# Jiraiya812/Fast-CU-Decision-HEVC

Measured on AMD Instinct MI355X. Metric: CTUs/sec (RDO decision only) at 4K all-intra, higher is better.
Workload: dtype int32+f64

## Files before the change

### __graft_entry__.py

```python
import importlib.util
import os
import subprocess
import sys

ROOT = os.path.dirname(os.path.abspath(__file__))
PKG_DIR = os.path.join(ROOT, "fast-cu-decision-hevc_amd")
PKG_NAME = "fast_cu_decision_hevc_amd"


def load_package():
    if PKG_NAME in sys.modules:
        return sys.modules[PKG_NAME]
    spec = importlib.util.spec_from_file_location(PKG_NAME, os.path.join(PKG_DIR, "__init__.py"),
                                                  submodule_search_locations=[PKG_DIR])
    mod = importlib.util.module_from_spec(spec)
    sys.modules[PKG_NAME] = mod
    spec.loader.exec_module(mod)
    return mod


REQUIRED_FLAG = "-amdgpu-remove-redundant-endcf=false"
ENGINE_FLAGS = ["--offload-arch=gfx950", "-std=c++17", "-O3", "-ffp-contract=off", "-fPIC", "-shared",
                "-DFCU_WAVES_PER_EU=4", "-Wno-unused-value", "-mllvm", REQUIRED_FLAG]

# ... 31 lines not shown
    hipcc = os.environ.get("HIPCC", "/opt/rocm/bin/hipcc")
    digest = _stale(lib, [p for p in srcs if not p.endswith("__graft_entry__.py")], ENGINE_FLAGS)
    if digest is not None:
        _run([hipcc] + ENGINE_FLAGS + ['-DFCU_BUILD_FLAGS="%s"' % " ".join(ENGINE_FLAGS),
                        "-o", lib, os.path.join(csrc, "fcu_kernels.hip")], csrc)
        with open(lib + ".stamp", "w") as f:
            f.write(digest)
        import ctypes
        info = ctypes.CDLL(lib).fcu_build_info
        info.restype = ctypes.c_char_p
        if REQUIRED_FLAG not in info().decode():
            raise RuntimeError("libfcu.so was built without %s: %s" % (REQUIRED_FLAG, info().decode()))
    _run(["make", "-s"], os.path.join(ROOT, "oracle"))
    emu = os.path.join(ROOT, "tests", "emu")
    shared = [p for p in [os.path.join(emu, "picture_emu.h")] if os.path.exists(p)]
    for name in ("fcu_emu", "dbk_emu", "sao_emu", "wpp_emu", "tiles_emu", "lf_tiles_emu", "lf_slices_emu", "report_emu", "host_emu", "hash_emu", "maps_emu", "labels_emu", "cu_trace_emu"):
        if not os.path.exists(os.path.join(emu, name + ".cpp")):
            continue
        if _newer(os.path.join(emu, "lib%s.so" % name), srcs + shared + [os.path.join(emu, name + ".cpp")]):
            _run(["g++", "-std=c++17", "-O2", "-fPIC", "-ffp-contract=off", "-shared", "-o", "lib%s.so" % name, name + ".cpp"], emu)
    orc = os.path.join(ROOT, "oracle")
    ref_srcs = [os.path.join(emu, "lf_tile_ref.c")] + [os.path.join(orc, f) for f in ("hmo_sao.c", "hmo_tables.c", "hmo.h", "hmo_int.h")]
    if _newer(os.path.join(emu, "liblf_tile_ref.so"), ref_srcs):
        _run(["gcc", "-O2", "-std=c11", "-fPIC", "-ffp-contract=off", "-fno-fast-math", "-shared", "-o", "liblf_tile_ref.so",
              "lf_tile_ref.c", os.path.join(orc, "hmo_tables.c"), "-lm"], emu)
    ref_srcs = [os.path.join(emu, "lf_slice_ref.c")] + [os.path.join(orc, f) for f in ("hmo_sao.c", "hmo_deblock.c", "hmo_tables.c", "hmo.h", "hmo_int.h")]
    if os.path.exists(ref_srcs[0]) and _newer(os.path.join(emu, "liblf_slice_ref.so"), ref_srcs):
        _run(["gcc", "-O2", "-std=c11", "-fPIC", "-ffp-contract=off", "-fno-fast-math", "-shared", "-o", "liblf_slice_ref.so",
              "lf_slice_ref.c", os.path.join(orc, "hmo_tables.c"), "-lm"], emu)
    ref_mk = os.path.join(ROOT, "oracle", "ref", "build_ref.sh")
    if os.path.isdir("/root/reference") and os.path.exists(ref_mk):
# ... 60 lines not shown
```

### fast-cu-decision-hevc_amd/csrc/fcu_engine.h

```cpp
#pragma once
#include <stdint.h>
#include <string.h>
#include <type_traits>
#include "../../include/fcu.h"

#ifdef FCU_EMU
#include <math.h>
#include <stdio.h>
#include <stdlib.h>
#define FCU_DEV static inline
#define FCU_MEMBER inline
#define FCU_NOINLINE
#define FCU_INLINE
#define FCU_TABLE static const
static int g_emu_phase = 0, g_emu_in_phase = 0, g_emu_lane = 0, g_emu_relax = 0;
#define FCU_EMU_RELAX(on) (g_emu_relax = (on))
static inline int fcu_emu_phase_begin() { g_emu_phase++; g_emu_in_phase = 1; g_emu_lane = 0; return 0; }
static inline int fcu_emu_phase_next(int lane) { if (lane + 1 >= 64) g_emu_in_phase = 0; g_emu_lane = lane + 1; return lane + 1; }
template <class T> static inline T fcu_emu_uni(T v, int site, int line)
{
  enum { SITES = 2048, K = 32, B = 16 };
  struct Seen { int phase, first, cur, idx, n; unsigned char vals[K][B]; };
  static Seen seen[SITES];
  if (g_emu_in_phase && !g_emu_relax && sizeof(T) <= B && site < SITES) {
    Seen &s = seen[site];
    if (s.phase != g_emu_phase) { s.phase = g_emu_phase; s.first = s.cur = g_emu_lane; s.idx = 0; s.n = 0; }
    if (s.cur != g_emu_lane) { s.cur = g_emu_lane; s.idx = 0; }
    if (g_emu_lane == s.first) { if (s.n < K) memcpy(s.vals[s.n++], &v, sizeof(T)); }
    else if (s.idx < s.n && memcmp(s.vals[s.idx], &v, sizeof(T)) != 0) { fprintf(stderr, "FCU_UNI at line %d: value differs between lanes of one phase\n", line); abort(); }
    s.idx++;
  }
  return v;
}
#define FCU_FOR_LANES for (int lane = fcu_emu_phase_begin(); lane < 64; lane = fcu_emu_phase_next(lane))
#define FCU_ATOMIC_ADD(p, v) (*(p) += (v))
#define FCU_ATOMIC_MAX(p, v) do { if (*(p) < (v)) *(p) = (v); } while (0)
#define FCU_ATOMIC_OR(p, v) (*(p) |= (v))
#define FCU_WAVE_ADD(p, v) (*(p) += (v))
#define FCU_WAVE_MIN64(p, v) do { if ((v) < *(p)) *(p) = (v); } while (0)
#define FCU_IN_LDS(p) do { } while (0)
#define FCU_UNI(x) fcu_emu_uni((x), __COUNTER__, __LINE__)
#define FCU_HBM
#define FCU_FLOOR(x) floor(x)
#define FCU_CHECK(c) do { if (!(c)) { fprintf(stderr, "FCU_CHECK failed: %s (line %d)\n", #c, __LINE__); abort(); } } while (0)
static unsigned long long g_emu_cu_paths[3] = { 0, 0, 0 };
#else
#define FCU_DEV __device__ static
#define FCU_MEMBER __device__ inline
#define FCU_NOINLINE __noinline__
#define FCU_INLINE __attribute__((always_inline))
#define FCU_TABLE __device__ static const
#define FCU_FOR_LANES for (int lane = (int)threadIdx.x, fcu_once_ = 1; fcu_once_; fcu_once_ = 0, __syncthreads())
#define FCU_ATOMIC_ADD(p, v) atomicAdd((p), (v))
#define FCU_ATOMIC_MAX(p, v) atomicMax((p), (v))
#define FCU_ATOMIC_OR(p, v) atomicOr((p), (v))
__device__ inline uint32_t fcu_wave_sum(uint32_t v)
{
  v += (uint32_t)__builtin_amdgcn_update_dpp(0, (int)v, 0xb1, 0xf, 0xf, false);
  v += (uint32_t)__builtin_amdgcn_update_dpp(0, (int)v, 0x4e, 0xf, 0xf, false);
  v += (uint32_t)__builtin_amdgcn_update_dpp(0, (int)v, 0x124, 0xf, 0xf, false);
  v += (uint32_t)__builtin_amdgcn_update_dpp(0, (int)v, 0x128, 0xf, 0xf, false);
  v += (uint32_t)__builtin_amdgcn_update_dpp(0, (int)v, 0x142, 0xa, 0xf, false);
  v += (uint32_t)__builtin_amdgcn_update_dpp(0, (int)v, 0x143, 0xc, 0xf, false);
  return (uint32_t)__builtin_amdgcn_readlane((int)v, 63);
}
__device__ inline unsigned long long fcu_wave_min64(unsigned long long v)
{
// ... 43 lines not shown
#define FCU_TOC(E_, v, idx) do { if ((idx) == 10 && threadIdx.x == 0) (E_).C->prof[idx] += (unsigned long long)(clock64() - v); } while (0)
#define FCU_COUNT(E_, idx, n) do { } while (0)
#elif defined(FCU_PROFILE_RDOQ) || defined(FCU_PROFILE_DEPTH)
#define FCU_TOC(E_, v, idx) do { if ((idx) < 11 && threadIdx.x == 0) (E_).C->prof[idx] += (unsigned long long)(clock64() - v); } while (0)
#define FCU_COUNT(E_, idx, n) do { } while (0)
#elif defined(FCU_PROFILE_RMD)
#define FCU_MTOC(E_, v, idx) do { if (threadIdx.x == 0) (E_).C->prof[idx] += (unsigned long long)(clock64() - v); } while (0)
#define FCU_TOC(E_, v, idx) do { if ((idx) < 11 && threadIdx.x == 0) (E_).C->prof[idx] += (unsigned long long)(clock64() - v); } while (0)
#define FCU_COUNT(E_, idx, n) do { } while (0)
#elif defined(FCU_PROFILE_CUSYN)
#define FCU_STOC(E_, v, idx) do { if (threadIdx.x == 0) (E_).C->prof[idx] += (unsigned long long)(clock64() - v); } while (0)
#define FCU_SPATH(E_, path) do { if (threadIdx.x == 0) (E_).C->prof[15] += 1ull << (21 * (path)); } while (0)
#define FCU_S7_COEFF(E_, v, comp) do { if (g_S.prof_s7 == 1) FCU_STOC(E_, v, (comp) ? 14 : 13); } while (0)
#define FCU_TOC(E_, v, idx) do { if ((idx) < 11 && threadIdx.x == 0) (E_).C->prof[idx] += (unsigned long long)(clock64() - v); } while (0)
#define FCU_COUNT(E_, idx, n) do { } while (0)
#else
#define FCU_TOC(E_, v, idx) do { if (threadIdx.x == 0) (E_).C->prof[idx] += (unsigned long long)(clock64() - v); } while (0)
#define FCU_COUNT(E_, idx, n) do { (E_).C->prof[idx] += (unsigned long long)(n); } while (0)
#endif
#else
#define FCU_TIC(v) do { } while (0)
#define FCU_TOC(E_, v, idx) do { } while (0)
#define FCU_COUNT(E_, idx, n) do { } while (0)
#endif
#ifndef FCU_QTOC
#define FCU_QTIC(v) do { } while (0)
#define FCU_QTOC(E_, v, idx) do { } while (0)
#endif
#ifndef FCU_ITOC
#define FCU_ITOC(E_, v, idx) do { } while (0)
#endif
#ifndef FCU_MTOC
#define FCU_MTOC(E_, v, idx) do { } while (0)
#endif
#ifndef FCU_STOC
#define FCU_STOC(E_, v, idx) do { } while (0)
#define FCU_SPATH(E_, path) do { } while (0)
#define FCU_S7_COEFF(E_, v, comp) do { } while (0)
#endif

#include "fcu_tables.h"

struct HotTables { uint32_t bin[256]; uint16_t scan[3][16]; uint8_t scan_cg8[3][4]; uint8_t ctx_ind_map4x4[16]; uint8_t group_idx[32];
                   uint64_t scan4_nib[3], map4_nib; uint32_t cnt_bits[4]; };
#ifdef FCU_EMU
static HotTables g_hot;
#else
__shared__ HotTables g_hot;
// ... 322 lines not shown
  }
  return first + offset;
}
FCU_DEV int coef_remain_bins(uint32_t symbol, uint32_t rparam)
{
  int code = (int)symbol;
  if (code < (3 << rparam)) return (int)(((uint32_t)code >> rparam) + 1) + (int)rparam;
  uint32_t length = rparam;
  code -= 3 << rparam;
  while (code >= (1 << length)) code -= 1 << (length++);
  return (int)(3 + length + 1 - rparam) + (int)length;
}
#ifdef FCU_EMU
enum { WALK_RDOQ_CALLS, WALK_RDOQ_TOP_IS_GROUP0, WALK_RDOQ_AHEAD_GROUPS, WALK_RDOQ_ONLY_GROUP0, WALK_RDOQ_ONLY_LAST_GROUP, WALK_RDOQ_ALL_ZERO,
       WALK_BITS_CALLS, WALK_BITS_ONE_EMPTY_RUN_BETWEEN, WALK_BITS_SECOND_ROUND, WALK_N };
extern "C" { __attribute__((weak)) unsigned long long fcu_emu_walk_cnt[WALK_N]; }
static const int32_t *g_emu_lscan_lo = nullptr, *g_emu_lscan_hi = nullptr;
#define FCU_WALK_COUNT(i, n) (fcu_emu_walk_cnt[i] += (unsigned long long)(n))
#define FCU_CHECK_LSCAN(p) FCU_CHECK((const int32_t *)(p) >= g_emu_lscan_lo && (const int32_t *)(p) < g_emu_lscan_hi)
#else
#define FCU_WALK_COUNT(i, n) do { } while (0)
#define FCU_CHECK_LSCAN(p) do { } while (0)
#endif
template <int SER>
FCU_DEV FCU_INLINE void code_coeff_body(int c, const int16_t *coef, int st, int last, int log2, int comp, int scanType, int tsFlag, const Params &P_, int16_t *absCoeff)
{
  if (SER) { c = FCU_UNI(c); coef = FCU_UNI(coef); last = FCU_UNI(last); scanType = FCU_UNI(scanType); tsFlag = FCU_UNI(tsFlag); absCoeff = FCU_UNI(absCoeff); }
  const Params &P = *FCU_UNI(&P_);
  st = FCU_UNI(st); log2 = FCU_UNI(log2); comp = FCU_UNI(comp);
  FCU_IN_LDS(absCoeff);
  const FCU_HBM int16_t *coefg = (const FCU_HBM int16_t *)coef;
  const int ch = comp ? 1 : 0, N = 1 << log2; int n2 = N * N;
  if (last < 0 && st == 1 && n2 >= 64) {
    int q = (n2 >> 6) - 1;
    for (; q >= 0; q--) {
      uint32_t w[32];
// ... 556 lines not shown
    for (int sp = 0; sp < n2 - 16; sp++) other |= dstg[sp * st];
    FCU_WALK_COUNT(WALK_RDOQ_ONLY_LAST_GROUP, !other);
  }
#endif
  return rdoq_finish<SER>(cb, P, srcg, dstg, recg, cgg, st, log2, ch, scanType, cbfCtx, scan, scanCG, cgflag, cgLastScanPos, lastScanPos, baseCost, blockUncodedCost, lambda);
}

#ifdef FCU_EMU
template <class T> struct LaneVar {
  T v[64];
  LaneVar() { for (int i = 0; i < 64; i++) v[i] = T(); }
  void set(int lane, T x) { v[lane] = x; }
  T own(int lane) const { return v[lane]; }
  T get(int k) const { return v[k]; }
  void put(int k, T x) { v[k] = x; }
};
FCU_DEV uint32_t lane_mask16(const LaneVar<int> &f) { uint32_t m = 0; for (int k = 0; k < 16; k++) m |= (uint32_t)(f.v[k] != 0) << k; return m; }
#else
#if defined(__HIP_DEVICE_COMPILE__)
#define FCU_READLANE(v, k) __builtin_amdgcn_readlane((v), (k))
#define FCU_WRITELANE(val_, k_, old_) (((int)threadIdx.x == (k_)) ? (val_) : (old_))
#define FCU_BALLOT(p) __builtin_amdgcn_ballot_w64(p)
#else
#define FCU_READLANE(v, k) (v)
#define FCU_WRITELANE(val_, k_, old_) (val_)
#define FCU_BALLOT(p) ((unsigned long long)(p))
#endif
template <class T> struct LaneVar;
template <> struct LaneVar<int> {
  int r = 0;
  __device__ void set(int, int x) { r = x; }
  __device__ int own(int) const { return r; }
  __device__ int get(int k) const { return FCU_READLANE(r, k); }
  __device__ void put(int k, int x) { r = FCU_WRITELANE(x, k, r); }
};
template <> struct LaneVar<double> {
  double r = 0;
  __device__ void set(int, double x) { r = x; }
  __device__ double own(int) const { return r; }
  __device__ double get(int k) const
  { union { double d; int i[2]; } u; u.d = r; u.i[0] = FCU_READLANE(u.i[0], k); u.i[1] = FCU_READLANE(u.i[1], k); return u.d; }
  __device__ void put(int k, double x)
  { union { double d; int i[2]; } u, w; u.d = r; w.d = x; u.i[0] = FCU_WRITELANE(w.i[0], k, u.i[0]); u.i[1] = FCU_WRITELANE(w.i[1], k, u.i[1]); r = u.d; }
};
__device__ inline uint32_t lane_mask16(const LaneVar<int> &f) { return (uint32_t)FCU_BALLOT(f.r != 0) & 0xffffu; }
#endif

#ifndef FCU_WAVE_RDOQ_MIN_LOG2
#define FCU_WAVE_RDOQ_MIN_LOG2 2
// ... 389 lines not shown
FCU_DEV int tr_index(int i, int log2) { const int N = 1 << log2; return ((i & (N - 1)) << log2) + (i >> log2); }
template <int LOG2> FCU_DEV int32_t fwd1(const int16_t *resi, int useDst, int idx)
{ constexpr int N = 1 << LOG2, s1 = LOG2 - 1; const int k = idx >> LOG2, y = idx & (N - 1); return (dot_row<N>(basis_row<LOG2>(useDst, k), resi + (y << LOG2)) + (1 << (s1 - 1))) >> s1; }
template <int LOG2> FCU_DEV int32_t fwd2(const int32_t *tmp, int useDst, int idx)
{ constexpr int N = 1 << LOG2, s2 = LOG2 + 6; const int k2 = idx >> LOG2, k1 = idx & (N - 1); return (dot_row<N>(basis_row<LOG2>(useDst, k2), tmp + (k1 << LOG2)) + (1 << (s2 - 1))) >> s2; }
template <int LOG2> FCU_DEV int32_t inv1(const int32_t *deqT, int useDst, int idx)
{ constexpr int N = 1 << LOG2; const int y = idx >> LOG2, kh = idx & (N - 1); return clip3i(-32768, 32767, (dot_row<N>(basis_col<LOG2>(useDst, y), deqT + (kh << LOG2)) + 64) >> 7); }
template <int LOG2> FCU_DEV int32_t inv2(const int32_t *tmp2, int useDst, int idx)
{ constexpr int N = 1 << LOG2; const int y = idx >> LOG2, x = idx & (N - 1); return clip3i(-32768, 32767, (dot_row<N>(basis_col<LOG2>(useDst, x), tmp2 + (y << LOG2)) + 2048) >> 12); }
template <int LOG2> FCU_DEV int32_t fwd1(RowCache<(1 << LOG2), int16_t> &rc, const int16_t *resi, int useDst, int idx)
{ constexpr int N = 1 << LOG2, s1 = LOG2 - 1; const int k = idx >> LOG2, y = idx & (N - 1); return (dot_regs<N>(basis_row<LOG2>(useDst, k), rc.get(resi + (y << LOG2))) + (1 << (s1 - 1))) >> s1; }
template <int LOG2> FCU_DEV int32_t fwd2(RowCache<(1 << LOG2), int32_t> &rc, const int32_t *tmp, int useDst, int idx)
{ constexpr int N = 1 << LOG2, s2 = LOG2 + 6; const int k2 = idx >> LOG2, k1 = idx & (N - 1); return (dot_regs<N>(basis_row<LOG2>(useDst, k2), rc.get(tmp + (k1 << LOG2))) + (1 << (s2 - 1))) >> s2; }
template <int LOG2> FCU_DEV int32_t inv1(RowCache<(1 << LOG2), int32_t> &rc, const int32_t *deqT, int useDst, int idx)
{ constexpr int N = 1 << LOG2; const int y = idx >> LOG2, kh = idx & (N - 1); return clip3i(-32768, 32767, (dot_regs<N>(basis_col<LOG2>(useDst, y), rc.get(deqT + (kh << LOG2))) + 64) >> 7); }
struct DeqParams { int scale, rs, lo, hi; };
FCU_DEV DeqParams deq_params(int log2, int qp)
{
  DeqParams d;
  const int per = qp / 6, rem = qp % 6;
  d.rs = 6 - ((15 - 8 - log2) + per); d.scale = k_inv_quant_scales[rem];
  int tbd = 32 + d.rs - 7; if (tbd > 16) tbd = 16;
  d.lo = -(1 << (tbd - 1)); d.hi = (1 << (tbd - 1)) - 1;
  return d;
}
FCU_DEV int32_t dequant1(int q, const DeqParams &d)
{
  const int c = clip3i(d.lo, d.hi, q);
  if (d.rs > 0) return clip3i(-32768, 32767, (c * d.scale + (1 << (d.rs - 1))) >> d.rs);
  return clip3i(-32768, 32767, (c * d.scale) << (-d.rs));
// ... 313 lines not shown
  FCU_TIC(t11_);
  const int d = cu->depth_cu, N = comp ? tu.cw : (1 << tu.log2), log2 = ilog2(N), n2 = N * N;
  const int bx = comp ? tu.cx : tu.x, by = comp ? tu.cy : tu.y, bs = comp ? 32 : 64, sh = comp ? 1 : 0;
  const int part = tu.part, layer = LOG2_MAXTU - tu.log2;
  uint8_t *org = yuv_plane(&G->org[d], comp) + by * bs + bx;
  uint8_t *pred = yuv_plane(&G->predt[d], comp) + by * bs + bx;
  uint8_t *recqt = yuv_plane(&G->qt_rec[layer], comp) + by * bs + bx;
  const int px = (cu->x >> sh) + bx, py = (cu->y >> sh) + by;
  uint8_t *recpic = E.C->rec[comp] + py * E.C->stride[comp] + px; const int rs = E.C->stride[comp];
  int16_t *coef = G->qt_coef[comp][layer] + (comp ? tu.off_c : tu.off_y);
  const int useTS = cu->tskip[comp][part];
  const int mode = comp ? chroma_final_mode(cu, part) : cu->intra_dir[0][part];
  const int useDst = comp == 0 && log2 == 2;
  const int qp = comp ? P.qp_c : P.qp;

  if (save1load2 != 2) {
    const int filt = use_filtered_ref(mode, log2, comp == 0);
    build_ref(comp, px, py, log2, filt);
    FCU_FOR_LANES {
      const uint8_t *r = filt ? g_S.reff : g_S.ref; const int dc = g_S.dc;
      if (lane == 0) g_S.t_last = -1;
      for (int i = lane; i < n2; i += 64) {
        const int y = i >> log2, x = i & (N - 1);
        const int v = pred_pixel(r, log2, mode, comp == 0, dc, x, y);
        pred[y * bs + x] = (uint8_t)v;
        if (save1load2 == 1) G->shared_pred[comp][i] = (uint8_t)v;
        G->p_resi[i] = (int16_t)(org[y * bs + x] - v);
      }
    }
  } else {
    FCU_FOR_LANES {
      if (lane == 0) g_S.t_last = -1;
      for (int i = lane; i < n2; i += 64) {
        const int y = i >> log2, x = i & (N - 1); const int v = G->shared_pred[comp][i];
        pred[y * bs + x] = (uint8_t)v; G->p_resi[i] = (int16_t)(org[y * bs + x] - v);
      }
    }
  }
  const int scanType = coef_scan_idx(mode, log2, comp), qbits = rdoq_qbits(log2, qp), qscale = k_quant_scales[qp % 6];
  const uint16_t *iscan = k_iscan + k_scan_off[scanType * 4 + log2 - 2];
  if (useTS) { FCU_FOR_LANES { est_build(cab, lane); for (int i = lane; i < n2; i += 64) { const int sp = iscan[i]; const int32_t ld = level_double((int32_t)G->p_resi[i] << (15 - 8 - log2), qscale, qbits); G->p_lscan[sp] = ld; if (level_nonzero(ld, qbits)) FCU_ATOMIC_MAX(&g_S.t_last, sp); } } }
  else {
    FCU_FOR_LANES { by_log2(log2, [&](auto L) { constexpr int LG = decltype(L)::value; RowCache<(1 << LG), int16_t> rc; for (int i = lane; i < n2; i += 64) G->p_tmp[i] = fwd1<LG>(rc, G->p_resi, useDst, i); }); }
    FCU_FOR_LANES { est_build(cab, lane); by_log2(log2, [&](auto L) { constexpr int LG = decltype(L)::value; RowCache<(1 << LG), int32_t> rc; for (int i = lane; i < n2; i += 64) { const int sp = iscan[i]; const int32_t ld = level_double(fwd2<LG>(rc, G->p_tmp, useDst, i), qscale, qbits); G->p_lscan[sp] = ld; if (level_nonzero(ld, qbits)) FCU_ATOMIC_MAX(&g_S.t_last, sp); } }); }
  }
  {
    FCU_TIC(t8_);
    const int cbfCtx = comp ? (CTX_CBF_CHROMA + tu.tr_depth) : (CTX_CBF_LUMA + (tu.tr_depth == 0 ? 1 : 0));
    const int useRdoq = FCU_UNI((int)(useTS ? P.rdoq_ts : P.rdoq));
    const int onWave = useRdoq && log2 >= FCU_WAVE_RDOQ_MIN_LOG2;
    if (onWave) rdoq_wave(cab, G->p_lscan, G->p_qscan, FCU_UNI(g_S.t_last), log2, comp, scanType, cbfCtx, P, G->r_rec, G->r_cg);
    FCU_FOR_LANES {
      if (comp == 0) for (int i = lane; i < tu.nparts; i += 64) cu->tr_idx[part + i] = (uint8_t)tu.tr_depth;
      if (lane == 0) {
        if (onWave) { g_S.t_abs = g_S.rw_abs; g_S.t_lsp = g_S.rw_lsp; }
        else if (useRdoq) { const RdoqOut o = rdoq<1, 1>(cab, G->p_lscan, G->p_qscan, 1, g_S.t_last, log2, comp, scanType, cbfCtx, P, G->r_rec, G->r_cg); g_S.t_abs = o.abs_sum; g_S.t_lsp = o.last; }
        else { const RdoqOut o = quant_plain(G->p_lscan, G->p_qscan, 1, g_S.t_last, log2, comp, P); g_S.t_abs = o.abs_sum; g_S.t_lsp = o.last; }
        E.C->n_tu_trials++;
        FCU_COUNT(E, 15, (1ull << 40) + (unsigned long long)(g_S.t_last >= 0 ? ((g_S.t_last >> 4) + 1) * 16 : 0));
      }
    }
    FCU_TOC(E, t8_, 8);
  }
  const int absSum = g_S.t_abs;
  FCU_FOR_LANES {
    const int np = comp ? tu_nparts_c(tu) : tu.nparts;
    for (int i = lane; i < np; i += 64) cu->cbf[comp][part + i] = (uint8_t)((absSum > 0 ? 1 : 0) << tu.tr_depth);
    const int cgEnd = ((g_S.t_last >> 4) + 1) << 4;
    const DeqParams dq = deq_params(log2, qp);
    for (int i = lane; i < n2; i += 64) { const int sp = iscan[i]; const int q = (absSum > 0 && sp < cgEnd) ? G->p_qscan[sp] : 0; coef[sp] = (int16_t)q; G->p_tmp[useTS ? i : tr_index(i, log2)] = dequant1(q, dq); }
  }
  if (absSum > 0) {
    if (useTS) { FCU_FOR_LANES { const int s = 15 - 8 - log2; for (int i = lane; i < n2; i += 64) G->p_resi[i] = (int16_t)((G->p_tmp[i] + (1 << (s - 1))) >> s); } }
    else {
      FCU_FOR_LANES { by_log2(log2, [&](auto L) { constexpr int LG = decltype(L)::value; RowCache<(1 << LG), int32_t> rc; for (int i = lane; i < n2; i += 64) G->p_tcoef[i] = inv1<LG>(rc, G->p_tmp, useDst, i); }); }
      FCU_FOR_LANES { by_log2(log2, [&](auto L) { for (int i = lane; i < n2; i += 64) G->p_resi[i] = (int16_t)inv2<decltype(L)::value>(G->p_tcoef, useDst, i); }); }
    }
  }
  FCU_FOR_LANES {
    if (lane == 0) g_S.sad[35] = 0;
  }
  FCU_FOR_LANES {
    uint32_t sse = 0;
    for (int i = lane; i < n2; i += 64) {
      const int y = i >> log2, x = i & (N - 1);
      const int r = clip8(pred[y * bs + x] + (absSum > 0 ? G->p_resi[i] : 0));
      pred[y * bs + x] = (uint8_t)r; recqt[y * bs + x] = (uint8_t)r; recpic[y * rs + x] = (uint8_t)r;
      const int e = org[y * bs + x] - r; sse += (uint32_t)(e * e);
    }
    FCU_WAVE_ADD(&g_S.sad[35], sse);
  }
  FCU_SERIAL { const uint32_t sse = g_S.sad[35]; g_S.t_dist = comp ? (uint32_t)(P.chroma_weight * (double)sse) : sse; }
  FCU_TOC(E, t11_, 11);
}

FCU_DEV FCU_NOINLINE void store_intra_result_qt(uint32_t tu_k, int comp)
{
  const Env E = env_get(); const TU tu = tu_of_key(FCU_UNI(tu_k)); comp = FCU_UNI(comp);
  Scratch *G = E.G;
  if (comp && tu.cw == 0) return;
  const int N = comp ? tu.cw : (1 << tu.log2), layer = LOG2_MAXTU - tu.log2, bs = comp ? 32 : 64, bx = comp ? tu.cx : tu.x, by = comp ? tu.cy : tu.y;
  const int16_t *src = G->qt_coef[comp][layer] + (comp ? tu.off_c : tu.off_y);
  const uint8_t *s = yuv_plane(&G->qt_rec[layer], comp) + by * bs + bx; uint8_t *t = yuv_plane(&G->ts_rec, comp) + by * bs + bx;
  FCU_FOR_LANES { for (int i = lane; i < N * N; i += 64) { G->ts_coef[comp][i] = src[i]; t[(i / N) * bs + (i % N)] = s[(i / N) * bs + (i % N)]; } }
}
FCU_DEV FCU_NOINLINE void load_intra_result_qt(const CuObj *cu, uint32_t tu_k, int comp)
{
// ... 28 lines not shown
        FCU_FOR_LANES { for (int i = lane; i < tu.nparts; i += 64) cu->tskip[0][part + i] = (uint8_t)modeId; }
        tu_trial(cu, tu_key(tu), 0, (CAB_GOON), modeId == 0 ? 1 : 2);
        const uint32_t tmpDist = FCU_UNI(g_S.t_dist), tmpCbf = FCU_UNI((uint32_t)((cu->cbf[0][part] >> trDepth) & 1));
        double tmpCost;
        if (modeId == 1 && tmpCbf == 0) tmpCost = FCU_MAX_DOUBLE;
        else {
          { FCU_TIC(t12_); FCU_SERIAL { const uint64_t f0 = g_S.cab[CAB_GOON].frac & 32767; g_S.vc_bits[0] = leaf_luma_bits(CAB_GOON, cu, tu_key(tu)); g_S.t_frac = g_S.cab[CAB_GOON].frac - f0; g_S.t_bins = g_S.cab[CAB_GOON].bins; } FCU_TOC(E, t12_, 12); }
          tmpCost = FCU_UNI(rd_cost(P, g_S.vc_bits[0], tmpDist));
        }
        if (tmpCost < singleCost) {
          singleCost = tmpCost; singleDist = tmpDist; singleCbf = tmpCbf; bestModeId = modeId; singleFrac = FCU_UNI(g_S.t_frac); singleBins = FCU_UNI(g_S.t_bins);
          if (bestModeId == 0) { store_intra_result_qt(tu_key(tu), 0); FCU_FOR_LANES cab_copy(slot_ptr(E, fullDepth, CI_TEMP_BEST), &g_S.cab[CAB_GOON], lane); }
        }
        if (modeId == 0) FCU_FOR_LANES cab_copy(&g_S.cab[CAB_GOON], slot_ptr(E, fullDepth, CI_QT_TRAFO_ROOT), lane);
      }
      FCU_FOR_LANES { for (int i = lane; i < tu.nparts; i += 64) cu->tskip[0][part + i] = (uint8_t)bestModeId; }
      if (bestModeId == 0) {
        load_intra_result_qt(cu, tu_key(tu), 0);
        FCU_FOR_LANES { for (int i = lane; i < tu.nparts; i += 64) cu->cbf[0][part + i] = (uint8_t)(singleCbf << trDepth); cab_copy(&g_S.cab[CAB_GOON], slot_ptr(E, fullDepth, CI_TEMP_BEST), lane); }
      }
    } else {
      if (checkSplit) FCU_FOR_LANES cab_copy(slot_ptr(E, fullDepth, CI_QT_TRAFO_ROOT), &g_S.cab[CAB_GOON], lane);
      FCU_FOR_LANES { for (int i = lane; i < tu.nparts; i += 64) cu->tskip[0][part + i] = 0; }
      if (reuseVc >= 0) {
        const int bv = reuseVc, N = 1 << log2, n2 = N * N, layer = LOG2_MAXTU - log2, cbf = FCU_UNI((int)(g_S.vc_abs[bv] > 0));
        FCU_SERIAL { const Cabac *w = &g_S.cab[CAB_LANE0 + g_S.vc_slot[bv]]; g_S.t_frac = w->frac - (g_S.cab[CAB_GOON].frac & 32767); g_S.t_bins = w->bins; }
        singleFrac = FCU_UNI(g_S.t_frac); singleBins = FCU_UNI(g_S.t_bins);
        FCU_FOR_LANES {
          for (int i = lane; i < n2; i += 64) {
            G->qt_coef[0][layer][tu.off_y + i] = (cbf && (i >> 4) <= (g_S.vc_last[bv] >> 4)) ? G->p_qscan[i * g_S.pu_nvc + bv] : (int16_t)0;
// ... 292 lines not shown
    g_S.n_rd = numFull;
  }
  FCU_MTOC(E, tm2_, 13);
}

FCU_DEV FCU_NOINLINE void pu_first_pass_batched(CuObj *cu, uint32_t tu_k)
{
  const Env E = env_get(); cu = FCU_UNI(cu); const TU tu = tu_of_key(FCU_UNI(tu_k));
  Scratch *G = E.G; const Params &P = E.C->p;
  const int d = cu->depth_cu, N = 1 << tu.log2, log2 = tu.log2, n2 = N * N, part = tu.part;
  const int partSize = cu->part_size[part];
  int checkTS = P.transform_skip && log2 == 2;
  if (P.ts_fast) checkTS = checkTS && (partSize == SIZE_NxN);
  const int nc = g_S.n_rd, tsv = checkTS ? 2 : 1, tss = tsv - 1, nvc = nc * tsv;
  FCU_CHECK(nvc <= MAXVC && nvc * n2 <= POOL && (MAXLC % 2) == 0);
  const int qbits = rdoq_qbits(log2, P.qp), qscale = k_quant_scales[P.qp % 6];
  const int useDst = log2 == 2;
  const uint8_t *org = G->org[d].y + tu.y * 64 + tu.x;
  const int haveRefs = FCU_UNI(g_S.ref_tag) == ref_key(cu->x + tu.x, cu->y + tu.y, log2);
  if (!haveRefs) { FCU_TIC(tm_); build_ref(0, cu->x + tu.x, cu->y + tu.y, log2, 1); FCU_MTOC(E, tm_, 14); }
  FCU_FOR_LANES {
    if (lane == 0) g_S.ref_tag = -1;
    const int dc = g_S.dc;
    for (int i = lane; i < nc * n2; i += 64) {
      const int cnd = i / n2, p = i - cnd * n2, y = p >> log2, x = p & (N - 1), mode = g_S.rd_mode[cnd];
      const uint8_t *r = use_filtered_ref(mode, log2, 1) ? g_S.reff : g_S.ref;
      const int v = pred_pixel(r, log2, mode, 1, dc, x, y);
      G->p_pred[i] = (uint8_t)v; G->p_resi[i] = (int16_t)(org[y * 64 + x] - v);
    }
  }
  FCU_FOR_LANES { if (lane < nvc) g_S.vc_last[lane] = -1; by_log2(log2, [&](auto L) { constexpr int LG = decltype(L)::value; RowCache<(1 << LG), int16_t> rc; for (int i = lane; i < nc * n2; i += 64) { const int cnd = i / n2; G->p_tmp[i] = fwd1<LG>(rc, G->p_resi + cnd * n2, useDst, i - cnd * n2); } }); }
  FCU_FOR_LANES {
    est_build(CAB_CUR0 + d, lane);
    by_log2(log2, [&](auto L) { constexpr int LG = decltype(L)::value; RowCache<(1 << LG), int32_t> rc;
      for (int i = lane; i < nvc * n2; i += 64) {
        const int v = i / n2, p = i - v * n2, cnd = (v >> tss), ts = (v & tss);
        const uint16_t *iscan = k_iscan + k_scan_off[coef_scan_idx(g_S.rd_mode[cnd], log2, 0) * 4 + log2 - 2];
        const int32_t t = ts ? ((int32_t)G->p_resi[cnd * n2 + p] << (15 - 8 - log2)) : fwd2<LG>(rc, G->p_tmp + cnd * n2, useDst, p);
        const int sp = iscan[p]; const int32_t ld = level_double(t, qscale, qbits);
        G->p_lscan[sp * nvc + v] = ld;
        if (level_nonzero(ld, qbits)) FCU_ATOMIC_MAX(&g_S.vc_last[v], sp);
      }
    });
  }
  FCU_TIC(t2_);
  FCU_FOR_LANES {
    if (lane < nvc) {
      const int mode = g_S.rd_mode[(lane >> tss)];
      RdoqRec *rrec = G->r_rec + lane; double *rcg = G->r_cg + lane;
      const int cbfCtx = CTX_CBF_LUMA + (tu.tr_depth == 0 ? 1 : 0);
      const RdoqOut o = ((lane & tss) ? P.rdoq_ts : P.rdoq) ? rdoq<0, 1>(CAB_CUR0 + d, G->p_lscan + lane, G->p_qscan + lane, nvc, g_S.vc_last[lane], log2, 0, coef_scan_idx(mode, log2, 0), cbfCtx, P, rrec, rcg, lane)
                                                            : quant_plain(G->p_lscan + lane, G->p_qscan + lane, nvc, g_S.vc_last[lane], log2, 0, P);
      g_S.vc_abs[lane] = o.abs_sum; g_S.vc_lsp[lane] = o.last;
      g_S.vc_dist[lane] = 0;
    }
    if (lane == 0) E.C->n_tu_trials += (unsigned long long)nvc;
  }
  FCU_TOC(E, t2_, 2);
  FCU_FOR_LANES {
    const DeqParams dq = deq_params(log2, P.qp);
    for (int i = lane; i < nvc * n2; i += 64) {
      const int v = i / n2, p = i - v * n2;
      const uint16_t *iscan = k_iscan + k_scan_off[coef_scan_idx(g_S.rd_mode[(v >> tss)], log2, 0) * 4 + log2 - 2];
      const int sp = iscan[p];
      const int q = (g_S.vc_abs[v] > 0 && (sp >> 4) <= (g_S.vc_last[v] >> 4)) ? G->p_qscan[sp * nvc + v] : 0;
      G->p_tmp[((v & tss)) ? i : v * n2 + tr_index(p, log2)] = dequant1(q, dq);
    }
  }
  FCU_FOR_LANES {
    by_log2(log2, [&](auto L) { constexpr int LG = decltype(L)::value; RowCache<(1 << LG), int32_t> rc;
      for (int i = lane; i < nvc * n2; i += 64) {
        const int v = i / n2, p = i - v * n2, ts = (v & tss);
        if (ts) { const int s = 15 - 8 - log2; G->p_tcoef[i] = (G->p_tmp[i] + (1 << (s - 1))) >> s; }
// ... 3 lines not shown
  }
  FCU_FOR_LANES {
    by_log2(log2, [&](auto L) {
      uint32_t acc = 0;
      for (int i = lane; i < nvc * n2; i += 64) {
        const int v = i / n2, p = i - v * n2, cnd = (v >> tss), ts = (v & tss), y = p >> log2, x = p & (N - 1);
        int res = 0;
        if (g_S.vc_abs[v] > 0) res = ts ? (int16_t)G->p_tcoef[i] : inv2<decltype(L)::value>(G->p_tcoef + v * n2, useDst, p);
        const int r = clip8(G->p_pred[cnd * n2 + p] + res);
        G->p_rec[i] = (uint8_t)r;
        const int e = org[y * 64 + x] - r;
        FCU_DIST_ADD(acc, v, e, i, n2);
      }
    });
  }
  FCU_TIC(t3_);
  for (int vbase = 0; vbase < nvc; vbase += MAXLC) {
    const int slotBase = vbase ? (g_S.vc_slot[g_S.pu_best_vc] + 1) % MAXLC : 0;
#if defined(FCU_EMU) && defined(FCU_EMU_TRACE_ROUNDS)
    if (vbase) fprintf(stderr, "second bit-count round: %d variants\n", nvc);
#endif
    FCU_WALK_COUNT(WALK_BITS_SECOND_ROUND, vbase != 0);
    FCU_FOR_LANES {
      const int vc = vbase + lane;
      if (lane < MAXLC && vc < nvc) {
        const int cnd = (vc >> tss), ts = (vc & tss), mode = g_S.rd_mode[cnd], cbf = g_S.vc_abs[vc] > 0;
        const int slot = (slotBase + lane) % MAXLC;
        double cost;
        g_S.vc_slot[vc] = (uint8_t)slot;
        if (ts && !cbf) cost = FCU_MAX_DOUBLE;
// ... 16 lines not shown
    }
    FCU_SERIAL {
      const int ncDone = ((vbase + MAXLC < nvc) ? vbase + MAXLC : nvc) / tsv;
      double best = FCU_MAX_DOUBLE; int bv = 0;
      for (int cnd = 0; cnd < ncDone; cnd++) {
        int v = cnd * tsv; double c = g_S.vc_cost[v];
        if (tsv == 2 && g_S.vc_cost[v + 1] < c) { v = v + 1; c = g_S.vc_cost[v]; }
        if (c < best) { best = c; bv = v; }
      }
      g_S.pu_nvc = nvc; g_S.pu_best_vc = bv; g_S.pu_best_cost = best; g_S.pu_best_dist = g_S.vc_dist[bv]; g_S.pu_best_mode = g_S.rd_mode[(bv >> tss)];
    }
  }
  FCU_TOC(E, t3_, 3);
  {
    const int bv = g_S.pu_best_vc, ts = (bv & tss), cbf = g_S.vc_abs[bv] > 0;
    Yuv *reco = &G->reco[d][1 - g_S.reco_best_idx[d]];
    FCU_FOR_LANES {
      for (int i = lane; i < n2; i += 64) {
        cu->coef[0][tu.off_y + i] = (cbf && (i >> 4) <= (g_S.vc_last[bv] >> 4)) ? G->p_qscan[i * nvc + bv] : (int16_t)0;
        reco->y[(tu.y + (i >> log2)) * 64 + tu.x + (i & (N - 1))] = G->p_rec[bv * n2 + i];
      }
      for (int i = lane; i < tu.nparts; i += 64) { G->tmp_tr_idx[i] = (uint8_t)tu.tr_depth; G->tmp_cbf[i] = (uint8_t)(cbf << tu.tr_depth); G->tmp_tskip[i] = (uint8_t)ts; }
    }
  }
}

FCU_DEV FCU_NOINLINE void pu_first_pass_64(CuObj *cu, uint32_t root_k)
{
  const Env E = env_get(); cu = FCU_UNI(cu); const TU root = tu_of_key(FCU_UNI(root_k));
  Scratch *G = E.G; const Params &P = E.C->p;
// ... 267 lines not shown
  return cab_bits(c);
}

FCU_DEV FCU_NOINLINE void chroma_leaf_trials(CuObj *cu, uint32_t tu_k)
{
  const Env E = env_get(); cu = FCU_UNI(cu); const TU tu = tu_of_key(FCU_UNI(tu_k));
  Scratch *G = E.G; const Params &P = E.C->p;
  const int d = cu->depth_cu;
  const int N = tu.cw, log2 = ilog2(N), n2 = N * N, trDepth = tu.tr_depth;
  int checkTS = P.transform_skip && N <= 4;
  if (P.ts_fast) {
    checkTS = checkTS && (tu.log2 == 2);
    if (checkTS) { int nb = 0; const int maxp = tu.part + (tu.c_code_all ? 1 : 4); for (int p = tu.part; p < maxp; p++) nb += cu->tskip[0][p]; checkTS = checkTS && (nb > 0); }
  }
  const int tsv = checkTS ? 2 : 1, tss = tsv - 1;
  const int perRound = (tsv == 1 && 10 * n2 <= POOL) ? 2 : 1;
  const int nm = 5 * perRound, nvc = nm * tsv;
  const int qbits = rdoq_qbits(log2, P.qp_c), qscale = k_quant_scales[P.qp_c % 6];
  const int subPart = tu_part_c(tu), nPartsC = tu_nparts_c(tu);
  const int lumaDir = cu->intra_dir[0][tu.part & ~3];
  for (int comp0 = 1; comp0 < 3; comp0 += perRound) {
    const int px = (cu->x >> 1) + tu.cx, py = (cu->y >> 1) + tu.cy;
    for (int cc = 0; cc < perRound; cc++) {
      const int comp = comp0 + cc;
      const uint8_t *org = yuv_plane(&G->org[d], comp) + tu.cy * 32 + tu.cx;
      chroma_leaf_refs5(E, cu, comp, px, py, log2);
      FCU_FOR_LANES {
        for (int i = lane; i < 5 * n2; i += 64) {
          const int m = i / n2, p = i - m * n2, y = p >> log2, x = p & (N - 1);
          const int mode = g_S.c_modes[m] == DM_CHROMA ? lumaDir : g_S.c_modes[m];
// ... 699 lines not shown
```

Baseline: 20310.

## Compute small-TU luma transforms in registers via lane permutes instead of LDS pools

For 4x4 and 8x8 luma TU batch trials, the forward and inverse DCT/DST are now computed with each lane holding one coefficient and exchanging data through ds_bpermute. This replaces staging the intermediate rows in shared scratch pools with a barrier between passes, and removes the barriers inside these phases. It also skips the inverse transform for all-zero 8x8 blocks. The change adds profiling and counter macros that compile to nothing by default, and it costs more permute instructions per dot product.

```diff
diff --git a/__graft_entry__.py b/__graft_entry__.py
--- a/__graft_entry__.py
+++ b/__graft_entry__.py
@@ -69,7 +69,7 @@
     _run(["make", "-s"], os.path.join(ROOT, "oracle"))
     emu = os.path.join(ROOT, "tests", "emu")
     shared = [p for p in [os.path.join(emu, "picture_emu.h")] if os.path.exists(p)]
-    for name in ("fcu_emu", "dbk_emu", "sao_emu", "wpp_emu", "tiles_emu", "lf_tiles_emu", "lf_slices_emu", "report_emu", "host_emu", "hash_emu", "maps_emu", "labels_emu", "cu_trace_emu"):
+    for name in ("fcu_emu", "fcu_emu_pools", "dbk_emu", "sao_emu", "wpp_emu", "tiles_emu", "lf_tiles_emu", "lf_slices_emu", "report_emu", "host_emu", "hash_emu", "maps_emu", "labels_emu", "cu_trace_emu"):
         if not os.path.exists(os.path.join(emu, name + ".cpp")):
             continue
         if _newer(os.path.join(emu, "lib%s.so" % name), srcs + shared + [os.path.join(emu, name + ".cpp")]):
diff --git a/fast-cu-decision-hevc_amd/csrc/fcu_engine.h b/fast-cu-decision-hevc_amd/csrc/fcu_engine.h
--- a/fast-cu-decision-hevc_amd/csrc/fcu_engine.h
+++ b/fast-cu-decision-hevc_amd/csrc/fcu_engine.h
@@ -33,6 +33,7 @@
   return v;
 }
 #define FCU_FOR_LANES for (int lane = fcu_emu_phase_begin(); lane < 64; lane = fcu_emu_phase_next(lane))
+#define FCU_FOR_LANES_REG FCU_FOR_LANES
 #define FCU_ATOMIC_ADD(p, v) (*(p) += (v))
 #define FCU_ATOMIC_MAX(p, v) do { if (*(p) < (v)) *(p) = (v); } while (0)
 #define FCU_ATOMIC_OR(p, v) (*(p) |= (v))
@@ -51,6 +52,7 @@
 #define FCU_INLINE __attribute__((always_inline))
 #define FCU_TABLE __device__ static const
 #define FCU_FOR_LANES for (int lane = (int)threadIdx.x, fcu_once_ = 1; fcu_once_; fcu_once_ = 0, __syncthreads())
+#define FCU_FOR_LANES_REG for (int lane = (int)threadIdx.x, fcu_once_ = 1; fcu_once_; fcu_once_ = 0)
 #define FCU_ATOMIC_ADD(p, v) atomicAdd((p), (v))
 #define FCU_ATOMIC_MAX(p, v) atomicMax((p), (v))
 #define FCU_ATOMIC_OR(p, v) atomicOr((p), (v))
@@ -124,6 +126,13 @@
 #define FCU_S7_COEFF(E_, v, comp) do { if (g_S.prof_s7 == 1) FCU_STOC(E_, v, (comp) ? 14 : 13); } while (0)
 #define FCU_TOC(E_, v, idx) do { if ((idx) < 11 && threadIdx.x == 0) (E_).C->prof[idx] += (unsigned long long)(clock64() - v); } while (0)
 #define FCU_COUNT(E_, idx, n) do { } while (0)
+#elif defined(FCU_PROFILE_PIX)
+#define FCU_PTIC(v) long long v = clock64()
+#define FCU_PRST(v) (v = clock64())
+#define FCU_PIX_SLOT(part, log2) ((int)((0x0fedcb976543ull >> (4 * ((part) * 3 + ((log2) >= 4 ? 2 : (log2) - 2)))) & 15))
+#define FCU_PTOC(E_, v, idx) do { if (threadIdx.x == 0) (E_).C->prof[idx] += (unsigned long long)(clock64() - v); v = clock64(); } while (0)
+#define FCU_TOC(E_, v, idx) do { if (((idx) == 1 || (idx) == 2 || (idx) == 8 || (idx) == 10) && threadIdx.x == 0) (E_).C->prof[idx] += (unsigned long long)(clock64() - v); } while (0)
+#define FCU_COUNT(E_, idx, n) do { } while (0)
 #else
 #define FCU_TOC(E_, v, idx) do { if (threadIdx.x == 0) (E_).C->prof[idx] += (unsigned long long)(clock64() - v); } while (0)
 #define FCU_COUNT(E_, idx, n) do { (E_).C->prof[idx] += (unsigned long long)(n); } while (0)
@@ -142,6 +151,11 @@
 #endif
 #ifndef FCU_MTOC
 #define FCU_MTOC(E_, v, idx) do { } while (0)
+#endif
+#ifndef FCU_PTOC
+#define FCU_PTIC(v) do { } while (0)
+#define FCU_PRST(v) do { } while (0)
+#define FCU_PTOC(E_, v, idx) do { } while (0)
 #endif
 #ifndef FCU_STOC
 #define FCU_STOC(E_, v, idx) do { } while (0)
@@ -494,12 +508,15 @@
 #ifdef FCU_EMU
 enum { WALK_RDOQ_CALLS, WALK_RDOQ_TOP_IS_GROUP0, WALK_RDOQ_AHEAD_GROUPS, WALK_RDOQ_ONLY_GROUP0, WALK_RDOQ_ONLY_LAST_GROUP, WALK_RDOQ_ALL_ZERO,
        WALK_BITS_CALLS, WALK_BITS_ONE_EMPTY_RUN_BETWEEN, WALK_BITS_SECOND_ROUND, WALK_N };
-extern "C" { __attribute__((weak)) unsigned long long fcu_emu_walk_cnt[WALK_N]; }
+enum { SMALL_TS_WINNER, SMALL_ALL_ZERO, SMALL_BATCH_OVER_16, SMALL_CHROMA_4X4, SMALL_N };
+extern "C" { __attribute__((weak)) unsigned long long fcu_emu_walk_cnt[WALK_N]; __attribute__((weak)) unsigned long long fcu_emu_small_cnt[SMALL_N]; }
+#define FCU_SMALL_COUNT(i, n) (fcu_emu_small_cnt[i] += (unsigned long long)(n))
 static const int32_t *g_emu_lscan_lo = nullptr, *g_emu_lscan_hi = nullptr;
 #define FCU_WALK_COUNT(i, n) (fcu_emu_walk_cnt[i] += (unsigned long long)(n))
 #define FCU_CHECK_LSCAN(p) FCU_CHECK((const int32_t *)(p) >= g_emu_lscan_lo && (const int32_t *)(p) < g_emu_lscan_hi)
 #else
 #define FCU_WALK_COUNT(i, n) do { } while (0)
+#define FCU_SMALL_COUNT(i, n) do { } while (0)
 #define FCU_CHECK_LSCAN(p) do { } while (0)
 #endif
 template <int SER>
@@ -1086,6 +1103,7 @@
   T own(int lane) const { return v[lane]; }
   T get(int k) const { return v[k]; }
   void put(int k, T x) { v[k] = x; }
+  T from(int src) const { return v[src & 63]; }
 };
 FCU_DEV uint32_t lane_mask16(const LaneVar<int> &f) { uint32_t m = 0; for (int k = 0; k < 16; k++) m |= (uint32_t)(f.v[k] != 0) << k; return m; }
 #else
@@ -1093,10 +1111,12 @@
 #define FCU_READLANE(v, k) __builtin_amdgcn_readlane((v), (k))
 #define FCU_WRITELANE(val_, k_, old_) (((int)threadIdx.x == (k_)) ? (val_) : (old_))
 #define FCU_BALLOT(p) __builtin_amdgcn_ballot_w64(p)
+#define FCU_PERMUTE(v, src) __builtin_amdgcn_ds_bpermute((src) << 2, (v))
 #else
 #define FCU_READLANE(v, k) (v)
 #define FCU_WRITELANE(val_, k_, old_) (val_)
 #define FCU_BALLOT(p) ((unsigned long long)(p))
+#define FCU_PERMUTE(v, src) (v)
 #endif
 template <class T> struct LaneVar;
 template <> struct LaneVar<int> {
@@ -1105,6 +1125,7 @@
   __device__ int own(int) const { return r; }
   __device__ int get(int k) const { return FCU_READLANE(r, k); }
   __device__ void put(int k, int x) { r = FCU_WRITELANE(x, k, r); }
+  __device__ int from(int src) const { return FCU_PERMUTE(r, src); }
 };
 template <> struct LaneVar<double> {
   double r = 0;
@@ -1524,6 +1545,30 @@
 { constexpr int N = 1 << LOG2, s2 = LOG2 + 6; const int k2 = idx >> LOG2, k1 = idx & (N - 1); return (dot_regs<N>(basis_row<LOG2>(useDst, k2), rc.get(tmp + (k1 << LOG2))) + (1 << (s2 - 1))) >> s2; }
 template <int LOG2> FCU_DEV int32_t inv1(RowCache<(1 << LOG2), int32_t> &rc, const int32_t *deqT, int useDst, int idx)
 { constexpr int N = 1 << LOG2; const int y = idx >> LOG2, kh = idx & (N - 1); return clip3i(-32768, 32767, (dot_regs<N>(basis_col<LOG2>(useDst, y), rc.get(deqT + (kh << LOG2))) + 64) >> 7); }
+template <int N>
+FCU_DEV int32_t dot_lanes(const int8_t *m, const LaneVar<int> &a, int src0, int step)
+{
+  m = (const int8_t *)__builtin_assume_aligned(m, N);
+  uint32_t mw[N / 4];
+  __builtin_memcpy(mw, m, N);
+  int32_t s = 0;
+#pragma unroll
+  for (int n = 0; n < N; n++) s += (int32_t)(int8_t)(mw[n >> 2] >> (8 * (n & 3))) * a.from(src0 + n * step);
+  return s;
+}
+template <int LOG2> FCU_DEV int32_t fwd1_lanes(const LaneVar<int> &resi, int useDst, int blk, int idx)
+{ constexpr int N = 1 << LOG2, s1 = LOG2 - 1; const int k = idx >> LOG2, y = idx & (N - 1); return (dot_lanes<N>(basis_row<LOG2>(useDst, k), resi, blk + (y << LOG2), 1) + (1 << (s1 - 1))) >> s1; }
+template <int LOG2> FCU_DEV int32_t fwd2_lanes(const LaneVar<int> &tmp, int useDst, int blk, int idx)
+{ constexpr int N = 1 << LOG2, s2 = LOG2 + 6; const int k2 = idx >> LOG2, k1 = idx & (N - 1); return (dot_lanes<N>(basis_row<LOG2>(useDst, k2), tmp, blk + (k1 << LOG2), 1) + (1 << (s2 - 1))) >> s2; }
+template <int LOG2> FCU_DEV int32_t inv1_lanes(const LaneVar<int> &deq, int useDst, int blk, int idx)
+{ constexpr int N = 1 << LOG2; const int y = idx >> LOG2, kh = idx & (N - 1); return clip3i(-32768, 32767, (dot_lanes<N>(basis_col<LOG2>(useDst, y), deq, blk + kh, N) + 64) >> 7); }
+template <int LOG2> FCU_DEV int32_t inv2_lanes(const LaneVar<int> &tmp2, int useDst, int blk, int idx)
+{ constexpr int N = 1 << LOG2; const int y = idx >> LOG2, x = idx & (N - 1); return clip3i(-32768, 32767, (dot_lanes<N>(basis_col<LOG2>(useDst, x), tmp2, blk + (y << LOG2), 1) + 2048) >> 12); }
+#ifdef FCU_SMALL_TU_POOLS
+#define FCU_SMALL_TU_REGS(log2) 0
+#else
+#define FCU_SMALL_TU_REGS(log2) ((log2) <= 3)
+#endif
 struct DeqParams { int scale, rs, lo, hi; };
 FCU_DEV DeqParams deq_params(int log2, int qp)
 {
@@ -1867,9 +1912,12 @@
   const int useDst = comp == 0 && log2 == 2;
   const int qp = comp ? P.qp_c : P.qp;
 
+  const int filt = use_filtered_ref(mode, log2, comp == 0);
+  if (save1load2 != 2) build_ref(comp, px, py, log2, filt);
+  FCU_PTIC(tp_);
+  const int scanType = coef_scan_idx(mode, log2, comp), qbits = rdoq_qbits(log2, qp), qscale = k_quant_scales[qp % 6];
+  const uint16_t *iscan = k_iscan + k_scan_off[scanType * 4 + log2 - 2];
   if (save1load2 != 2) {
-    const int filt = use_filtered_ref(mode, log2, comp == 0);
-    build_ref(comp, px, py, log2, filt);
     FCU_FOR_LANES {
       const uint8_t *r = filt ? g_S.reff : g_S.ref; const int dc = g_S.dc;
       if (lane == 0) g_S.t_last = -1;
@@ -1890,13 +1938,12 @@
       }
     }
   }
-  const int scanType = coef_scan_idx(mode, log2, comp), qbits = rdoq_qbits(log2, qp), qscale = k_quant_scales[qp % 6];
-  const uint16_t *iscan = k_iscan + k_scan_off[scanType * 4 + log2 - 2];
   if (useTS) { FCU_FOR_LANES { est_build(cab, lane); for (int i = lane; i < n2; i += 64) { const int sp = iscan[i]; const int32_t ld = level_double((int32_t)G->p_resi[i] << (15 - 8 - log2), qscale, qbits); G->p_lscan[sp] = ld; if (level_nonzero(ld, qbits)) FCU_ATOMIC_MAX(&g_S.t_last, sp); } } }
   else {
     FCU_FOR_LANES { by_log2(log2, [&](auto L) { constexpr int LG = decltype(L)::value; RowCache<(1 << LG), int16_t> rc; for (int i = lane; i < n2; i += 64) G->p_tmp[i] = fwd1<LG>(rc, G->p_resi, useDst, i); }); }
     FCU_FOR_LANES { est_build(cab, lane); by_log2(log2, [&](auto L) { constexpr int LG = decltype(L)::value; RowCache<(1 << LG), int32_t> rc; for (int i = lane; i < n2; i += 64) { const int sp = iscan[i]; const int32_t ld = level_double(fwd2<LG>(rc, G->p_tmp, useDst, i), qscale, qbits); G->p_lscan[sp] = ld; if (level_nonzero(ld, qbits)) FCU_ATOMIC_MAX(&g_S.t_last, sp); } }); }
   }
+  FCU_PTOC(E, tp_, FCU_PIX_SLOT(2, log2));
   {
     FCU_TIC(t8_);
     const int cbfCtx = comp ? (CTX_CBF_CHROMA + tu.tr_depth) : (CTX_CBF_LUMA + (tu.tr_depth == 0 ? 1 : 0));
@@ -1915,7 +1962,9 @@
     }
     FCU_TOC(E, t8_, 8);
   }
+  FCU_PRST(tp_);
   const int absSum = g_S.t_abs;
+  FCU_SMALL_COUNT(SMALL_ALL_ZERO, log2 <= 3 && absSum == 0); FCU_SMALL_COUNT(SMALL_CHROMA_4X4, comp != 0 && log2 == 2);
   FCU_FOR_LANES {
     const int np = comp ? tu_nparts_c(tu) : tu.nparts;
     for (int i = lane; i < np; i += 64) cu->cbf[comp][part + i] = (uint8_t)((absSum > 0 ? 1 : 0) << tu.tr_depth);
@@ -1944,6 +1993,7 @@
     FCU_WAVE_ADD(&g_S.sad[35], sse);
   }
   FCU_SERIAL { const uint32_t sse = g_S.sad[35]; g_S.t_dist = comp ? (uint32_t)(P.chroma_weight * (double)sse) : sse; }
+  FCU_PTOC(E, tp_, FCU_PIX_SLOT(3, log2));
   FCU_TOC(E, t11_, 11);
 }
 
@@ -2002,6 +2052,7 @@
         }
         if (modeId == 0) FCU_FOR_LANES cab_copy(&g_S.cab[CAB_GOON], slot_ptr(E, fullDepth, CI_QT_TRAFO_ROOT), lane);
       }
+      FCU_SMALL_COUNT(SMALL_TS_WINNER, bestModeId == 1);
       FCU_FOR_LANES { for (int i = lane; i < tu.nparts; i += 64) cu->tskip[0][part + i] = (uint8_t)bestModeId; }
       if (bestModeId == 0) {
         load_intra_result_qt(cu, tu_key(tu), 0);
@@ -2324,11 +2375,44 @@
   if (P.ts_fast) checkTS = checkTS && (partSize == SIZE_NxN);
   const int nc = g_S.n_rd, tsv = checkTS ? 2 : 1, tss = tsv - 1, nvc = nc * tsv;
   FCU_CHECK(nvc <= MAXVC && nvc * n2 <= POOL && (MAXLC % 2) == 0);
+  FCU_SMALL_COUNT(SMALL_BATCH_OVER_16, log2 == 2 && nvc > 16);
   const int qbits = rdoq_qbits(log2, P.qp), qscale = k_quant_scales[P.qp % 6];
   const int useDst = log2 == 2;
   const uint8_t *org = G->org[d].y + tu.y * 64 + tu.x;
   const int haveRefs = FCU_UNI(g_S.ref_tag) == ref_key(cu->x + tu.x, cu->y + tu.y, log2);
   if (!haveRefs) { FCU_TIC(tm_); build_ref(0, cu->x + tu.x, cu->y + tu.y, log2, 1); FCU_MTOC(E, tm_, 14); }
+  FCU_PTIC(tp_);
+  const int regs = FCU_SMALL_TU_REGS(log2), blk_mask = ~(n2 - 1), l2n2 = 2 * log2;
+  if (regs) {
+    FCU_FOR_LANES_REG { if (lane == 0) g_S.ref_tag = -1; if (lane < nvc) g_S.vc_last[lane] = -1; }
+    for (int base = 0; base < nc * n2; base += 64) {
+      LaneVar<int> vResi, vT1;
+      FCU_FOR_LANES_REG {
+        const int i = base + lane, act = i < nc * n2, cnd = act ? (i >> l2n2) : 0, p = i & (n2 - 1), y = p >> log2, x = p & (N - 1), mode = g_S.rd_mode[cnd];
+        const uint8_t *r = use_filtered_ref(mode, log2, 1) ? g_S.reff : g_S.ref;
+        const int v = pred_pixel(r, log2, mode, 1, g_S.dc, x, y);
+        int res = 0;
+        if (act) { G->p_pred[i] = (uint8_t)v; res = (int16_t)(org[y * 64 + x] - v); }
+        vResi.set(lane, res);
+      }
+      FCU_FOR_LANES_REG { vT1.set(lane, log2 == 2 ? fwd1_lanes<2>(vResi, useDst, lane & blk_mask, lane & (n2 - 1)) : fwd1_lanes<3>(vResi, 0, lane & blk_mask, lane & (n2 - 1))); }
+      FCU_FOR_LANES_REG {
+        const int i = base + lane, act = i < nc * n2, cnd = act ? (i >> l2n2) : 0, p = i & (n2 - 1);
+        const int32_t t = log2 == 2 ? fwd2_lanes<2>(vT1, useDst, lane & blk_mask, p) : fwd2_lanes<3>(vT1, 0, lane & blk_mask, p);
+        if (act) {
+          const uint16_t *iscan = k_iscan + k_scan_off[coef_scan_idx(g_S.rd_mode[cnd], log2, 0) * 4 + log2 - 2];
+          const int sp = iscan[p];
+          for (int ts = 0; ts < tsv; ts++) {
+            const int v = cnd * tsv + ts;
+            const int32_t ld = level_double(ts ? ((int32_t)vResi.own(lane) << (15 - 8 - log2)) : t, qscale, qbits);
+            G->p_lscan[sp * nvc + v] = ld;
+            if (level_nonzero(ld, qbits)) FCU_ATOMIC_MAX(&g_S.vc_last[v], sp);
+          }
+        }
+      }
+    }
+    FCU_FOR_LANES { est_build(CAB_CUR0 + d, lane); }
+  } else {
   FCU_FOR_LANES {
     if (lane == 0) g_S.ref_tag = -1;
     const int dc = g_S.dc;
@@ -2353,6 +2437,8 @@
       }
     });
   }
+  }
+  FCU_PTOC(E, tp_, FCU_PIX_SLOT(0, log2));
   FCU_TIC(t2_);
   FCU_FOR_LANES {
     if (lane < nvc) {
@@ -2367,6 +2453,42 @@
     if (lane == 0) E.C->n_tu_trials += (unsigned long long)nvc;
   }
   FCU_TOC(E, t2_, 2);
+  FCU_PRST(tp_);
+  if (regs) {
+    const DeqParams dq = deq_params(log2, P.qp);
+    for (int base = 0; base < nvc * n2; base += 64) {
+      const int skip = n2 == 64 && FCU_UNI(g_S.vc_abs[base >> 6]) == 0;
+      LaneVar<int> vDeq, vT2, vPO;
+      FCU_FOR_LANES_REG {
+        const int i = base + lane, act = i < nvc * n2, v = act ? (i >> l2n2) : 0, p = i & (n2 - 1), cnd = (v >> tss);
+        int dv = 0, po = 0;
+        if (act) {
+          const uint16_t *iscan = k_iscan + k_scan_off[coef_scan_idx(g_S.rd_mode[cnd], log2, 0) * 4 + log2 - 2];
+          const int sp = iscan[p];
+          const int q = (g_S.vc_abs[v] > 0 && (sp >> 4) <= (g_S.vc_last[v] >> 4)) ? G->p_qscan[sp * nvc + v] : 0;
+          dv = dequant1(q, dq);
+          po = G->p_pred[cnd * n2 + p] | (org[(p >> log2) * 64 + (p & (N - 1))] << 8);
+        }
+        vDeq.set(lane, dv); vPO.set(lane, po);
+      }
+      if (!skip) FCU_FOR_LANES_REG { vT2.set(lane, log2 == 2 ? inv1_lanes<2>(vDeq, useDst, lane & blk_mask, lane & (n2 - 1)) : inv1_lanes<3>(vDeq, 0, lane & blk_mask, lane & (n2 - 1))); }
+      FCU_FOR_LANES_REG {
+        const int i = base + lane, act = i < nvc * n2, v = act ? (i >> l2n2) : 0, p = i & (n2 - 1), ts = (v & tss);
+        const int t = skip ? 0 : (log2 == 2 ? inv2_lanes<2>(vT2, useDst, lane & blk_mask, p) : inv2_lanes<3>(vT2, 0, lane & blk_mask, p));
+        int e = 0;
+        if (act) {
+          int res = 0;
+          if (g_S.vc_abs[v] > 0) { const int s = 15 - 8 - log2; res = ts ? (int16_t)((vDeq.own(lane) + (1 << (s - 1))) >> s) : t; }
+          const int po = vPO.own(lane), r = clip8((po & 255) + res);
+          G->p_rec[i] = (uint8_t)r;
+          e = (po >> 8) - r;
+        }
+        if (n2 == 64) FCU_WAVE_ADD(&g_S.vc_dist[base >> 6], (uint32_t)(e * e));
+        else if (act) FCU_ATOMIC_ADD(&g_S.vc_dist[v], (uint32_t)(e * e));
+      }
+    }
+    FCU_FOR_LANES { }
+  } else {
   FCU_FOR_LANES {
     const DeqParams dq = deq_params(log2, P.qp);
     for (int i = lane; i < nvc * n2; i += 64) {
@@ -2400,6 +2522,8 @@
       }
     });
   }
+  }
+  FCU_PTOC(E, tp_, FCU_PIX_SLOT(1, log2));
   FCU_TIC(t3_);
   for (int vbase = 0; vbase < nvc; vbase += MAXLC) {
     const int slotBase = vbase ? (g_S.vc_slot[g_S.pu_best_vc] + 1) % MAXLC : 0;
@@ -2446,6 +2570,7 @@
   FCU_TOC(E, t3_, 3);
   {
     const int bv = g_S.pu_best_vc, ts = (bv & tss), cbf = g_S.vc_abs[bv] > 0;
+    FCU_SMALL_COUNT(SMALL_TS_WINNER, ts); FCU_SMALL_COUNT(SMALL_ALL_ZERO, log2 <= 3 && !cbf);
     Yuv *reco = &G->reco[d][1 - g_S.reco_best_idx[d]];
     FCU_FOR_LANES {
       for (int i = lane; i < n2; i += 64) {
@@ -2743,6 +2868,7 @@
     if (checkTS) { int nb = 0; const int maxp = tu.part + (tu.c_code_all ? 1 : 4); for (int p = tu.part; p < maxp; p++) nb += cu->tskip[0][p]; checkTS = checkTS && (nb > 0); }
   }
   const int tsv = checkTS ? 2 : 1, tss = tsv - 1;
+  FCU_SMALL_COUNT(SMALL_CHROMA_4X4, log2 == 2);
   const int perRound = (tsv == 1 && 10 * n2 <= POOL) ? 2 : 1;
   const int nm = 5 * perRound, nvc = nm * tsv;
   const int qbits = rdoq_qbits(log2, P.qp_c), qscale = k_quant_scales[P.qp_c % 6];
```

Result: faster. 20780, median of 6 (+2.3%).
